# huttered40/capital

Hardware: AMD Instinct MI355X
Metric: TFLOP/s (whole node) Cholesky n=65536, algorithmic n^3/3, recursive cholinv factor(), inputs resident in HBM (higher is better)
Workload: dtype f64

## Files before the change

### capital_amd/capi.py

```python
import ctypes as C
import os

import numpy as np
import torch

_HERE = os.path.dirname(os.path.abspath(__file__))
LIB_PATH = os.environ.get("CAPITAL_HIP_LIB", os.path.join(_HERE, "libcapital_hip.so"))

NOTRANS, TRANS = 0, 1
LEFT, RIGHT = 0, 1
LOWER, UPPER = 0, 1
NONUNIT, UNIT = 0, 1
RECT, UPPERTRI, LOWERTRI = 0, 1, 2

_i64, _dbl, _int, _vp = C.c_int64, C.c_double, C.c_int, C.c_void_p

_SIGS = {
    "capi_dgemm": [_int, _int, _i64, _i64, _i64, _dbl, _vp, _i64, _vp, _i64, _dbl, _vp, _i64],
    "capi_dsyrk": [_int, _int, _i64, _i64, _dbl, _vp, _i64, _dbl, _vp, _i64],
    "capi_dgemmt": [_int, _int, _int, _i64, _i64, _dbl, _vp, _i64, _vp, _i64, _dbl, _vp, _i64],
    "capi_dsyrk_panel32": [_i64, _i64, _dbl, _vp, _dbl, _vp, _i64],
    "capi_dtrmm_right_panel32": [_i64, _i64, _dbl, _vp, _i64, _vp, _i64, _vp, _i64],
    "capi_dtrmm": [_int, _int, _int, _int, _i64, _i64, _dbl, _vp, _i64, _vp, _i64],
    "capi_dtrmm_oop": [_int, _int, _int, _int, _i64, _i64, _dbl, _vp, _i64, _vp, _i64, _vp, _i64],
    "capi_dtrmm_acc": [_int, _int, _int, _int, _i64, _i64, _dbl, _vp, _i64, _vp, _i64, _dbl, _vp, _i64],
    "capi_dtrsm": [_int, _int, _int, _int, _i64, _i64, _dbl, _vp, _i64, _vp, _i64],
    "capi_dpotrf": [_int, _i64, _vp, _i64],
    "capi_dtrtri": [_int, _int, _i64, _vp, _i64],
    "capi_dpotrf_trtri": [_i64, _vp, _i64, _vp, _i64],
    "capi_dgram_equilibrate_shift": [_i64, _vp, _i64, _i64, _dbl, _vp, _vp],
    "capi_dtri_rescale": [_i64, _vp, _i64, _vp, _i64, _vp, _vp],
    "capi_dgemtn_ts": [_i64, _i64, _i64, _dbl, _vp, _i64, _vp, _i64, _dbl, _vp, _i64],
    "capi_dresid_ts": [_i64, _i64, _i64, _vp, _i64, _vp, _i64, _vp, _i64, _vp, _i64, _vp],
    "capi_dtrmm_thin": [_int, _int, _i64, _i64, _i64, _dbl, _vp, _i64, _i64, _vp, _i64, _dbl, _vp, _i64],
    "capi_dresid_sym": [_i64, _i64, _vp, _i64, _vp, _i64, _vp, _i64, _vp, _i64, _vp],
    "capi_get_info": [C.POINTER(_int)],
    "capi_reset_info": [],
    "capi_serialize": [_int, _int, _vp, _i64, _i64, _vp, _i64, _i64] + [_i64] * 8,
    "capi_serialize_shape": [_int, _int, _int, _vp, _i64, _i64, _vp, _i64, _i64] + [_i64] * 8,
    "capi_dlacpy": [_int, _i64, _i64, _vp, _i64, _vp, _i64],
    "capi_dgeadd": [_int, _i64, _i64, _dbl, _vp, _i64, _dbl, _vp, _i64],
    "capi_dtrizero": [_int, _i64, _vp, _i64],
    "capi_daxpby": [_i64, _dbl, _vp, _vp],
    "capi_remove_triangle": [C.c_char, _vp, _i64, _i64, _i64, _i64, _i64],
    "capi_block_to_cyclic": [_vp, _vp, _i64, _i64, _i64],
    "capi_block_to_cyclic_full": [_vp, _vp, _i64, _i64, _i64],
    "capi_cyclic_to_block": [_vp, _vp, _i64, _i64, _i64],
# ... 162 lines not shown
```

### capital_amd/csrc/gemm_f64.hip

```cpp
#include "capi_internal.h"
#include "gemm_plan.h"
#include <type_traits>

extern "C" int capi_internal_copy2d(capi_handle_t h, int64_t m, int64_t n, const double* A, int64_t lda, double* B, int64_t ldb);

typedef double d4_t __attribute__((ext_vector_type(4)));
typedef double d2_t __attribute__((ext_vector_type(2)));

namespace {

constexpr int NTHREADS = 256;
using gemm_plan::BK, gemm_plan::SK;
template <int TS> struct tile_cfg {
  static constexpr int TILE_LDS = TS * SK;
  static constexpr int STAGE_LDS = 2 * TILE_LDS;
  static constexpr int NQ = TS / 32;
  static constexpr int SUB = TS / 32;
};
constexpr int GROUP_M = 8;
template <int TS> __device__ __forceinline__ int rc_r(int tid, int q) { return 16 * ((tid >> 6) * (TS / 64) + (q >> 1)) + 2 * (tid & 7); }
__device__ __forceinline__ int rc_k(int tid, int q) { return 8 * (q & 1) + ((tid >> 3) & 7); }

struct GemmArgs {
  const double* A;
// ... 457 lines not shown
}

template <bool AK, bool BKC>
__global__ __launch_bounds__(NTHREADS, 2) void dtrmm_pair_kernel(const GemmArgs p) {
  constexpr int TS = 128, BM = TS, BN = TS, SUB = tile_cfg<TS>::SUB, NQ = tile_cfg<TS>::NQ;
  constexpr int NW = NQ * ((AK ? 1 : 2) + (BKC ? 1 : 2));
  constexpr int TILE_LDS = tile_cfg<TS>::TILE_LDS, STAGE_LDS = tile_cfg<TS>::STAGE_LDS;
  constexpr int kstep = BK;
  extern __shared__ __attribute__((aligned(16))) double lds[];
  const int tid = threadIdx.x;
  const int lane = tid & 63, wave = tid >> 6;
  const int r16 = lane & 15, g = lane >> 4;
  const int wm = wave & 1, wn = wave >> 1;
  stamp_begin(p);

  const int nblk = gridDim.x, bid = blockIdx.x;
  const int xcd = bid & 7, qq = nblk >> 3, rr = nblk & 7;
  const int pid = p.pid_base + (xcd < rr ? xcd * (qq + 1) : rr * (qq + 1) + (xcd - rr) * qq) + (bid >> 3);
  const bool left = p.tri_side == CAPI_LEFT;
  const int ntri = left ? p.tiles_m : p.tiles_n, nfree = left ? p.tiles_n : p.tiles_m, npair = ntri >> 1;
  int pb, fr;
  if (left) tile_of_dims(-1, npair, nfree, pid, pb, fr); else tile_of_dims(-1, nfree, npair, pid, fr, pb);
  const bool anchor0 = left ? !p.tri_eff_upper : (p.tri_eff_upper != 0);
  const bool maskA = left, maskB = !left;
  const bool keep_ge = left == (p.tri_eff_upper != 0);
  const int64_t ksa = AK ? kstep : (int64_t)kstep * p.lda, ksb = BKC ? kstep : (int64_t)kstep * p.ldb;
  const int64_t qsa = AK ? 32 * p.lda : 8 * p.lda;
  const int64_t qsa2 = AK ? 64 * p.lda : 16;
  const int64_t qsb = BKC ? 32 * p.ldb : 8 * p.ldb;
  const int64_t qsb2 = BKC ? 64 * p.ldb : 16;

  for (int ph = 0; ph < 2; ++ph) {
    const bool asc = (ph == 0) == anchor0;
    const int bt = asc ? pb : ntri - 1 - pb;
    const int ti = left ? bt : fr, tj = left ? fr : bt;
    const int i0 = ti * BM, j0 = tj * BN, d0 = left ? i0 : j0;
    const int klo = anchor0 ? 0 : d0, khi = anchor0 ? d0 + TS : p.K;
    const int ntk = (khi - klo) / kstep;
    const int tb0 = (d0 - klo) / BK, tb1 = tb0 + TS / BK;

    d4_t acc[SUB][SUB];
#pragma unroll
    for (int a = 0; a < SUB; ++a)
#pragma unroll
      for (int c = 0; c < SUB; ++c) acc[a][c] = (d4_t){0.0, 0.0, 0.0, 0.0};

    const double* const fa0 = AK ? p.A + (int64_t)(i0 + (tid >> 3)) * p.lda + klo + 2 * (tid & 7)
                              : p.A + (int64_t)(klo + rc_k(tid, 0)) * p.lda + i0 + rc_r<TS>(tid, 0);
    const double* const fb0 = BKC ? p.B + (int64_t)(j0 + (tid >> 3)) * p.ldb + klo + 2 * (tid & 7)
                              : p.B + (int64_t)(klo + rc_k(tid, 0)) * p.ldb + j0 + rc_r<TS>(tid, 0);
    const double* fa = fa0;
    const double* fb = fb0;
    const int64_t sa = asc ? ksa : -ksa, sb = asc ? ksb : -ksb;
    const int dir = asc ? 1 : -1;
    int t = asc ? 0 : ntk - 1;

    d2_t ra[NQ], rb[NQ];
    {
      const int kf = klo + t * kstep;
      panel_load<TS, AK>(p.A, p.lda, i0, p.M, kf, khi, tid, 1, ra);
      panel_load<TS, BKC>(p.B, p.ldb, j0, p.N, kf, khi, tid, 1, rb);
      if (maskA && t >= tb0 && t < tb1) panel_mask<TS, AK>(i0, kf, tid, keep_ge, p.tri_unit, ra);
// ... 859 lines not shown
  CAPI_REQUIRE(h, n >= 0 && k >= 0 && n < (1LL << 31) && k < (1LL << 31), "dims");
  if (n == 0) return CAPI_OK;
  CAPI_REQUIRE(h, C && ldc >= n, "C/ldc");
  if (k > 0) {
    CAPI_REQUIRE(h, A && B, "null operand");
    CAPI_REQUIRE(h, lda >= (transA ? k : n) && ldb >= (transB ? n : k), "lda/ldb");
  }
  GemmArgs p{};
  p.A = A; p.B = B; p.C = C; p.lda = lda; p.ldb = ldb; p.ldc = ldc;
  p.M = (int)n; p.N = (int)n; p.K = (int)k; p.alpha = alpha; p.beta = beta;
  p.out_uplo = uplo; p.tri_side = -1;
  return launch_gemm(h, transA == CAPI_TRANS, transB == CAPI_NOTRANS, p, true);
}

int capi_dsyrk(capi_handle_t h, int uplo, int trans, int64_t n, int64_t k, double alpha,
               const double* A, int64_t lda, double beta, double* C, int64_t ldc) {
  CAPI_REQUIRE(h, h, "null handle");
  CAPI_REQUIRE(h, ok01(trans), "transpose code");
  return capi_dgemmt(h, uplo, trans, trans == CAPI_TRANS ? CAPI_NOTRANS : CAPI_TRANS, n, k, alpha, A, lda, A, lda, beta, C, ldc);
}

static int trmm_launch(capi_handle_t h, int side, int uplo, int trans, int diag, int64_t m, int64_t n, double alpha,
                       const double* T, int64_t ldt, const double* B, int64_t ldb, double beta, double* C, int64_t ldc,
                       size_t ws_held = 0) {
  CAPI_REQUIRE(h, h, "null handle");
  CAPI_REQUIRE(h, ok01(side) && ok01(uplo) && ok01(trans) && ok01(diag), "enum code");
  CAPI_REQUIRE(h, m >= 0 && n >= 0 && m < (1LL << 31) && n < (1LL << 31), "dims");
  if (m == 0 || n == 0) return CAPI_OK;
  const int64_t nt = side == CAPI_LEFT ? m : n;
  CAPI_REQUIRE(h, T && B && C && ldt >= nt && ldb >= m && ldc >= m, "operands");
  CAPI_REQUIRE(h, (const double*)C != B, "out-of-place trmm: C aliases B");
  GemmArgs p{};
  p.C = C; p.ldc = ldc; p.M = (int)m; p.N = (int)n; p.K = (int)nt; p.alpha = alpha; p.beta = beta;
  p.out_uplo = -1;
  p.tri_side = side;
  p.tri_eff_upper = ((uplo == CAPI_UPPER) != (trans == CAPI_TRANS));
  p.tri_unit = diag == CAPI_UNIT;
  if (side == CAPI_RIGHT && diag == CAPI_NONUNIT && n >= 512 && n <= 4096 && m >= 64 * n) {
    void* w;
    int rc = capi_ws3_get(h, sizeof(double) * (size_t)n * (size_t)n, &w);
    if (rc != CAPI_OK) return rc;
    CAPI_HIP_CHECK(h, hipMemsetAsync(w, 0, sizeof(double) * (size_t)n * (size_t)n, h->stream));
    rc = capi_dlacpy(h, uplo == CAPI_UPPER ? 1 : 2, n, n, T, ldt, (double*)w, n);
    if (rc != CAPI_OK) return rc;
    T = (const double*)w;
    ldt = n;
    p.tri_dense = 1;
    const bool eff_upper = (uplo == CAPI_UPPER) != (trans == CAPI_TRANS);
    if (eff_upper && n % 256 == 0) {
      for (int64_t J = 0; J < n / 256; ++J) {
        GemmArgs q = p;
        q.N = 256;
        q.K = (int)(256 * (J + 1));
        q.tri_koff = (int)(256 * J);
        q.tri_block = 1;
        q.C = C + 256 * J * ldc;
        q.A = B; q.lda = ldb;
        q.B = trans == CAPI_NOTRANS ? T + 256 * J * ldt : T + 256 * J;
        q.ldb = ldt;
        int rc2 = launch_gemm(h, false, trans == CAPI_NOTRANS, q, ws_held == 0);
        if (rc2 != CAPI_OK) return rc2;
      }
      return CAPI_OK;
    }
  }
  if (side == CAPI_LEFT) {
    p.A = T; p.lda = ldt; p.B = B; p.ldb = ldb;
    return launch_gemm(h, trans == CAPI_TRANS, true, p, true, ws_held);
  } else {
    p.A = B; p.lda = ldb; p.B = T; p.ldb = ldt;
// ... 10 lines not shown
  const bool aligned = ((st | sb_ | sc_) & 1) == 0;
  if (batch > 1 && small_ok && aligned) {
    const int64_t nt = side == CAPI_LEFT ? m : n;
    GemmArgs p{};
    p.C = C; p.ldc = ldc; p.M = (int)m; p.N = (int)n; p.K = (int)nt; p.alpha = alpha; p.beta = 0.0;
    p.out_uplo = -1; p.tri_side = side;
    p.tri_eff_upper = ((uplo == CAPI_UPPER) != (trans == CAPI_TRANS));
    p.tri_unit = diag == CAPI_UNIT;
    p.batch = batch;
    if (side == CAPI_LEFT) { p.A = T; p.lda = ldt; p.sa = st; p.B = B; p.ldb = ldb; p.sb = sb_; p.sc = sc_; return launch_gemm(h, trans == CAPI_TRANS, true, p, true); }
    p.A = B; p.lda = ldb; p.sa = sb_; p.B = T; p.ldb = ldt; p.sb = st; p.sc = sc_;
    return launch_gemm(h, false, trans == CAPI_NOTRANS, p, true);
  }
  for (int b = 0; b < batch; ++b) {
    int rc = capi_dtrmm_oop(h, side, uplo, trans, diag, m, n, alpha, T + b * st, ldt, B + b * sb_, ldb, C + b * sc_, ldc);
    if (rc != CAPI_OK) return rc;
  }
  return CAPI_OK;
}

int capi_dtrmm_oop(capi_handle_t h, int side, int uplo, int trans, int diag, int64_t m, int64_t n, double alpha,
                   const double* T, int64_t ldt, const double* B, int64_t ldb, double* C, int64_t ldc) {
  return trmm_launch(h, side, uplo, trans, diag, m, n, alpha, T, ldt, B, ldb, 0.0, C, ldc);
}

int capi_dtrmm_acc(capi_handle_t h, int side, int uplo, int trans, int diag, int64_t m, int64_t n, double alpha,
                   const double* T, int64_t ldt, const double* B, int64_t ldb, double beta, double* C, int64_t ldc) {
  return trmm_launch(h, side, uplo, trans, diag, m, n, alpha, T, ldt, B, ldb, beta, C, ldc);
}

int capi_dtrmm(capi_handle_t h, int side, int uplo, int trans, int diag, int64_t m, int64_t n, double alpha,
               const double* T, int64_t ldt, double* B, int64_t ldb) {
  CAPI_REQUIRE(h, h, "null handle");
  if (m <= 0 || n <= 0) return m < 0 || n < 0 ? CAPI_EINVAL : CAPI_OK;
  void* ws;
  int rc = capi_ws_get(h, sizeof(double) * (size_t)m * (size_t)n, &ws);
  if (rc != CAPI_OK) return rc;
  rc = trmm_launch(h, side, uplo, trans, diag, m, n, alpha, T, ldt, B, ldb, 0.0, (double*)ws, m, (size_t)m * (size_t)n);
  if (rc != CAPI_OK) return rc;
  rc = capi_ws_get(h, sizeof(double) * (size_t)m * (size_t)n, &ws);
  if (rc != CAPI_OK) return rc;
  return capi_internal_copy2d(h, m, n, (const double*)ws, m, B, ldb);
}

int capi_dsyrk_panel32(capi_handle_t h, int64_t n, int64_t k, double alpha, const double* A32, double beta, double* C, int64_t ldc) {
  CAPI_REQUIRE(h, h, "null handle");
// ... 131 lines not shown
```

### capital_amd/csrc/gemm_plan.h

```cpp
#ifndef CAPITAL_GEMM_PLAN_H_
#define CAPITAL_GEMM_PLAN_H_

#include <cstddef>
#include <cstdint>
#include <cstdio>

#include "capital_hip.h"

namespace gemm_plan {

constexpr int BK = 16;
constexpr int SK = BK + 2;
constexpr int ST = 32, SKC = 256, SQK = 64, SLD = ST + 2;
constexpr int TSK_W = 256;

inline int64_t cdiv(int64_t a, int64_t b) { return (a + b - 1) / b; }

struct Product {
  int M = 0, N = 0, K = 0;
  int out_uplo = -1;
  int tri_side = -1;
  int tri_eff_upper = 0, tri_dense = 0, tri_block = 0, tri_koff = 0;
  bool alpha_zero = false;
  double beta = 0.0;
  int batch = 0;
  bool ak = false, bkc = false;
  bool a_is_b = false;
  bool same_ld = false;
  bool a_vec = false, b_vec = false;
  bool a_tiled = false, c_tiled = false;
  bool ws_for_slab = true;
};
struct Device { int num_cu = 256; int stream_cu = 0; };
struct Modes { int rounds_mode = 0, pair_mode = 1, pair_rounds = 0, pair_rounds_min = 0; };
struct Overrides { int force_ts = 0; int force_small = -1; };

enum class Path { none, scale, trmm_ts32, gram_blocks, gram_ts, small, tile, pair, refused };
enum class Reduce { none, narrow, wide };
inline const char* path_name(Path p) {
// ... 143 lines not shown
      r.k_per_split = (int)kps;
      r.k_rotate = !tri;
      r.slab_ld = p.M;
      r.slab_stride = (int64_t)p.M * p.N;
      r.reduce = Reduce::narrow;
    }
  }
  const int per_round = 2 * ncu;
  const bool use_rounds = r.ts == 128 && r.splitk == 1 && !tri && per_round % 16 == 0 && p.batch <= 1 && r.ntiles >= 2 * per_round &&
                          (p.out_uplo < 0 ? (mode.rounds_mode & 1) != 0 : ((mode.rounds_mode & 2) != 0 && r.order));
  if (r.ts == 128 && r.splitk == 1 && !tri) {
    const int rem = r.ntiles % per_round;
    if (r.ntiles >= 2 * per_round && rem > 0 && rem <= (3 * per_round) / 4) r.tail128 = rem;
  }
  const int ntiles_all = r.ntiles;
  r.ntiles -= r.tail128;
  r.blocks = (int64_t)r.ntiles * r.splitk;
  r.per_launch = use_rounds ? per_round : r.blocks;
  r.lds_bytes = sizeof(double) * 2 * 2 * (size_t)r.ts * SK;
  r.variant = vi + (r.ts == 128 ? 0 : 4);
  r.share_den = (double)ntiles_all * r.splitk;
  const int ntri = p.tri_side == CAPI_LEFT ? r.tiles_m : r.tiles_n, nfree = p.tri_side == CAPI_LEFT ? r.tiles_n : r.tiles_m;
  const int64_t wgs = (int64_t)(ntri / 2) * nfree;
  if (mode.pair_mode && tri && !p.tri_dense && !p.tri_block && p.tri_koff == 0 && r.ts == 128 && r.splitk == 1 && p.beta == 0.0 &&
      p.batch <= 1 && p.M % 128 == 0 && p.N % 128 == 0 && p.K % 128 == 0 && p.a_vec && p.b_vec && (ntri & 1) == 0 && wgs % per_round == 0 &&
      (mode.pair_mode > 1 || wgs <= 4 * per_round || (mode.pair_rounds && p.K >= mode.pair_rounds_min))) {
    r.path = Path::pair;
    r.blocks = wgs;
    r.per_launch = mode.pair_rounds && wgs > per_round && p.K >= mode.pair_rounds_min ? per_round : wgs;
    r.variant = vi + 16;
    r.share_den = (double)wgs;
  }
  return r;
}

inline int format(char* buf, size_t n, const Product& p, const Device& d, const Modes& m, const Overrides& o, const Plan& r) {
  static const char* const reduce_names[] = {"none", "narrow", "wide"};
  return snprintf(buf, n,
                  "M=%d N=%d K=%d out_uplo=%d tri_side=%d tri_eff_upper=%d tri_dense=%d tri_block=%d tri_koff=%d alpha_zero=%d beta=%.17g "
                  "batch=%d ak=%d bkc=%d a_is_b=%d same_ld=%d a_vec=%d b_vec=%d a_tiled=%d c_tiled=%d ws_for_slab=%d num_cu=%d stream_cu=%d "
                  "rounds_mode=%d pair_mode=%d pair_rounds=%d pair_rounds_min=%d force_ts=%d force_small=%d -> path=%s ts=%d splitk=%d "
                  "k_per_split=%d k_rotate=%d order=%d share_ab=%d slab_stride=%lld tiles_m=%d tiles_n=%d ntiles=%d blocks=%lld "
                  "per_launch=%lld launches=%lld grid_y=%d tail128=%d reduce=%s lds=%zu variant=%d share_den=%.17g est_us=%.1f small_est_us=%.1f",
                  p.M, p.N, p.K, p.out_uplo, p.tri_side, p.tri_eff_upper, p.tri_dense, p.tri_block, p.tri_koff, (int)p.alpha_zero, p.beta,
                  p.batch, (int)p.ak, (int)p.bkc, (int)p.a_is_b, (int)p.same_ld, (int)p.a_vec, (int)p.b_vec, (int)p.a_tiled, (int)p.c_tiled,
                  (int)p.ws_for_slab, d.num_cu, d.stream_cu, m.rounds_mode, m.pair_mode, m.pair_rounds, m.pair_rounds_min, o.force_ts,
                  o.force_small, path_name(r.path), r.ts, r.splitk, r.k_per_split, r.k_rotate, r.order, r.share_ab, (long long)r.slab_stride,
// ... 8 lines not shown
```

### capital_amd/csrc/movement.hip

```cpp
#include "capi_internal.h"

namespace {

__device__ __host__ inline int64_t st_offset(int st, int64_t x, int64_t y, int64_t dimY) {
  if (st == CAPI_RECT) return x * dimY + y;
  if (st == CAPI_UPPERTRI) return ((x * (x + 1)) >> 1) + y;
  return x * dimY + y - (x * (x + 1) / 2);
}

__global__ void serialize_kernel(int shape, int ss, int ds, const double* __restrict__ src, int64_t sdimY, double* __restrict__ dst,
                                 int64_t ddimY, int64_t ssx, int64_t ssy, int64_t dsx, int64_t dsy, int64_t rangeX,
                                 int64_t rangeY) {
  const int64_t y = (int64_t)blockIdx.x * 1024 + threadIdx.x;
  const bool lower = shape == CAPI_LOWERTRI, upper = shape == CAPI_UPPERTRI;
  for (int64_t i = blockIdx.y; i < rangeX; i += gridDim.y) {
    int64_t so, d_o, cnt;
    if (lower) {
      so = st_offset(ss, ssx + i, ssy + i, sdimY);
      d_o = st_offset(ds, dsx + i, dsy + i, ddimY);
      cnt = rangeY - i;
    } else {
      so = st_offset(ss, ssx + i, ssy, sdimY);
      d_o = st_offset(ds, dsx + i, dsy, ddimY);
      cnt = upper ? i + 1 : rangeY;
    }
    if (y >= cnt) continue;
    double v[4];
#pragma unroll
    for (int q = 0; q < 4; ++q) v[q] = src[so + (y + 256 * q < cnt ? y + 256 * q : y)];
#pragma unroll
    for (int q = 0; q < 4; ++q)
      if (y + 256 * q < cnt) dst[d_o + y + 256 * q] = v[q];
  }
}

__global__ void lacpy_kernel(int part, int64_t m, int64_t n, const double* __restrict__ A, int64_t lda, double* __restrict__ B,
                             int64_t ldb) {
  const int64_t i = (int64_t)blockIdx.x * blockDim.x + threadIdx.x;
  const int64_t j0 = (int64_t)blockIdx.y * 8;
  if (i >= m) return;
#pragma unroll
  for (int q = 0; q < 8; ++q) {
    const int64_t j = j0 + q;
    if (j >= n) break;
    if (part == 1 && i > j) continue;
    if (part == 2 && i < j) continue;
    B[i + j * ldb] = A[i + j * lda];
  }
}

typedef double d2m_t __attribute__((ext_vector_type(2)));
template <bool VEC>
__global__ __launch_bounds__(256) void copy2d_kernel(int64_t m, int64_t n, const double* __restrict__ A, int64_t lda, double* __restrict__ B, int64_t ldb) {
  const int64_t i = ((int64_t)blockIdx.x * 256 + threadIdx.x) * (VEC ? 2 : 1);
  if (i >= m) return;
  for (int64_t j0 = (int64_t)blockIdx.y * 8; j0 < n; j0 += (int64_t)gridDim.y * 8) {
    if (VEC) {
      d2m_t v[8];
#pragma unroll
      for (int q = 0; q < 8; ++q) v[q] = *(const d2m_t*)(A + i + (j0 + q < n ? j0 + q : j0) * lda);
#pragma unroll
      for (int q = 0; q < 8; ++q)
        if (j0 + q < n) *(d2m_t*)(B + i + (j0 + q) * ldb) = v[q];
    } else {
      double v[8];
#pragma unroll
      for (int q = 0; q < 8; ++q) v[q] = A[i + (j0 + q < n ? j0 + q : j0) * lda];
#pragma unroll
      for (int q = 0; q < 8; ++q)
        if (j0 + q < n) B[i + (j0 + q) * ldb] = v[q];
    }
  }
}

// ... 161 lines not shown

void pad_lens(int64_t dimX, int64_t dimY, int64_t gdimX, int64_t gdimY, int64_t px, int64_t py, int64_t PX, int64_t PY,
              int64_t* padX, int64_t* padY) {
  *padX = (((gdimX % PX != 0) && ((dimX - 1) * PX + px >= gdimX)) ? dimX - 1 : dimX);
  *padY = (((gdimY % PY != 0) && ((dimY - 1) * PY + py >= gdimY)) ? dimY - 1 : dimY);
}

inline dim3 grid2(int64_t rows, int64_t cols) { return dim3((unsigned)cdiv(rows, 256), (unsigned)(cols < 65535 ? cols : 65535)); }

}

extern "C" {

int capi_serialize_shape(capi_handle_t h, int shape, int ss, int ds, const double* src, int64_t sdimX, int64_t sdimY, double* dst,
                         int64_t ddimX, int64_t ddimY, int64_t ssx, int64_t sex, int64_t ssy, int64_t sey, int64_t dsx, int64_t dex,
                         int64_t dsy, int64_t dey) {
  CAPI_REQUIRE(h, h, "null handle");
  CAPI_REQUIRE(h, ss >= 0 && ss <= 2 && ds >= 0 && ds <= 2 && shape >= 0 && shape <= 2, "structure code");
  CAPI_REQUIRE(h, (sex - ssx) == (dex - dsx) && (sey - ssy) == (dey - dsy), "source and destination ranges differ");
  (void)sdimX; (void)ddimX;
  const int64_t rangeX = sex - ssx, rangeY = sey - ssy;
  if (rangeX <= 0 || rangeY <= 0) return CAPI_OK;
  CAPI_REQUIRE(h, src && dst, "null matrix");
  hipLaunchKernelGGL(serialize_kernel, dim3((unsigned)cdiv(rangeY, 1024), (unsigned)(rangeX < 65535 ? rangeX : 65535)), dim3(256), 0, h->stream, shape, ss, ds, src, sdimY, dst, ddimY, ssx, ssy,
                     dsx, dsy, rangeX, rangeY);
  CAPI_HIP_CHECK(h, hipGetLastError());
  return CAPI_OK;
}

int capi_serialize(capi_handle_t h, int ss, int ds, const double* src, int64_t sdimX, int64_t sdimY, double* dst, int64_t ddimX,
                   int64_t ddimY, int64_t ssx, int64_t sex, int64_t ssy, int64_t sey, int64_t dsx, int64_t dex, int64_t dsy,
                   int64_t dey) {
  const int shape = (ss == CAPI_LOWERTRI || ds == CAPI_LOWERTRI) ? CAPI_LOWERTRI : ((ss == CAPI_UPPERTRI || ds == CAPI_UPPERTRI) ? CAPI_UPPERTRI : CAPI_RECT);
  return capi_serialize_shape(h, shape, ss, ds, src, sdimX, sdimY, dst, ddimX, ddimY, ssx, sex, ssy, sey, dsx, dex, dsy, dey);
}

__attribute__((visibility("hidden"))) int capi_internal_copy2d(capi_handle_t h, int64_t m, int64_t n, const double* A, int64_t lda, double* B, int64_t ldb) {
  if (m <= 0 || n <= 0 || (A == B && lda == ldb)) return CAPI_OK;
  if (lda == m && ldb == m && m * n >= (1 << 16) && (m > 8192 || n == 1)) {
    const int64_t total = m * n, cols = total / 8192, rest = total - cols * 8192;
    int rc = capi_internal_copy2d(h, 8192, cols, A, 8192, B, 8192);
    if (rc != CAPI_OK || rest == 0) return rc;
    return capi_internal_copy2d(h, rest, 1, A + cols * 8192, rest, B + cols * 8192, rest);
  }
  const bool vec = (((uintptr_t)A | (uintptr_t)B) & 15) == 0 && ((lda | ldb | m) & 1) == 0;
  const int64_t gx = cdiv(vec ? m / 2 : m, 256), gy = cdiv(n, 8);
  CAPI_REQUIRE(h, gx < (1LL << 31), "copy too tall");
  const dim3 grid((unsigned)gx, (unsigned)(gy < 65535 ? gy : 65535));
  if (vec) hipLaunchKernelGGL(copy2d_kernel<true>, grid, dim3(256), 0, h->stream, m, n, A, lda, B, ldb);
  else hipLaunchKernelGGL(copy2d_kernel<false>, grid, dim3(256), 0, h->stream, m, n, A, lda, B, ldb);
  CAPI_HIP_CHECK(h, hipGetLastError());
  return CAPI_OK;
}

int capi_dlacpy(capi_handle_t h, int part, int64_t m, int64_t n, const double* A, int64_t lda, double* B, int64_t ldb) {
  CAPI_REQUIRE(h, h, "null handle");
  CAPI_REQUIRE(h, part >= 0 && part <= 2 && m >= 0 && n >= 0, "args");
  if (m == 0 || n == 0) return CAPI_OK;
  CAPI_REQUIRE(h, A && B && lda >= m && ldb >= m, "operands");
  if (part == 0) return capi_internal_copy2d(h, m, n, A, lda, B, ldb);
  const int64_t gy = cdiv(n, 8);
  CAPI_REQUIRE(h, gy <= 65535, "n too large");
  hipLaunchKernelGGL(lacpy_kernel, dim3((unsigned)cdiv(m, 256), (unsigned)gy), dim3(256), 0, h->stream, part, m, n, A, lda, B, ldb);
  CAPI_HIP_CHECK(h, hipGetLastError());
  return CAPI_OK;
}

int capi_dgeadd(capi_handle_t h, int part, int64_t m, int64_t n, double alpha, const double* X, int64_t ldx, double beta, double* Y,
                int64_t ldy) {
  CAPI_REQUIRE(h, h, "null handle");
  CAPI_REQUIRE(h, part >= 0 && part <= 2 && m >= 0 && n >= 0, "args");
  if (m == 0 || n == 0) return CAPI_OK;
  CAPI_REQUIRE(h, X && Y && ldx >= m && ldy >= m, "operands");
  hipLaunchKernelGGL(geadd_kernel, grid2(m, n), dim3(256), 0, h->stream, part, m, n, alpha, X, ldx, beta, Y, ldy);
  CAPI_HIP_CHECK(h, hipGetLastError());
  return CAPI_OK;
}

int capi_dtrizero(capi_handle_t h, int keep_uplo, int64_t n, double* A, int64_t lda) {
  CAPI_REQUIRE(h, h, "null handle");
  CAPI_REQUIRE(h, (keep_uplo == 0 || keep_uplo == 1) && n >= 0, "args");
  if (n == 0) return CAPI_OK;
  CAPI_REQUIRE(h, A && lda >= n, "A/lda");
  hipLaunchKernelGGL(trizero_kernel, grid2(n, n), dim3(256), 0, h->stream, keep_uplo, n, A, lda);
  CAPI_HIP_CHECK(h, hipGetLastError());
  return CAPI_OK;
// ... 128 lines not shown
```

### capital_amd/src/alg/cholesky/cholinv/cholinv.h

```cpp
#ifndef CAPITAL_CHOLESKY_CHOLINV_H_
#define CAPITAL_CHOLESKY_CHOLINV_H_

#include "./../../alg.h"
#include "./../../matmult/summa/summa.h"
#include "./policy.h"

#pragma weak capi_dtrmm_thin
#pragma weak capi_dresid_ts
#pragma weak capi_dresid_sym

namespace cholesky {

template <class SerializePolicy = policy::cholinv::Serialize, class IntermediatesPolicy = policy::cholinv::SaveIntermediates,
          class BaseCasePolicy = policy::cholinv::NoReplication>
class cholinv : public SerializePolicy, public IntermediatesPolicy, public BaseCasePolicy {
public:
  using SP = SerializePolicy;
  using IP = IntermediatesPolicy;
  using BP = BaseCasePolicy;

  template <typename ScalarT, typename DimensionT>
  class info {
  public:
    using ScalarType = ScalarT;
    using DimensionType = DimensionT;
    using alg_type = cholinv<SerializePolicy, IntermediatesPolicy, BaseCasePolicy>;
    using SP = SerializePolicy;
    using IP = IntermediatesPolicy;
    using BP = BaseCasePolicy;
    info(const info& p) : complete_inv(p.complete_inv), split(p.split), bc_mult_dim(p.bc_mult_dim), dir(p.dir) {}
// ... 406 lines not shown
    ++args.num_levels;
    const U split2 = localDim - split1;
    const bool single = (t.d == 1 && t.c == 1);
    matmult::arena& ws = args.work;
    view R11i{Ri + start + start * ld, ld, split1, split1};
    view A12{R + start + (start + split1) * ld, ld, split1, split2};
    view A22{R + (start + split1) + (start + split1) * ld, ld, split2, split2};
    view R22i{Ri + (start + split1) + (start + split1) * ld, ld, split2, split2};
    view I12{Ri + start + (start + split1) * ld, ld, split1, split2};

    invoke(args, t, R, Ri, ld, start, split1, globalDim >> 1);
    if (wait_ev >= 0) CAPITAL_CHECK(capi_event_wait(h, wait_ev));
    if (start == 0 && args.input_lead > 0 && split1 == args.input_lead) CAPITAL_CHECK(capi_event_wait(h, EV_INPUT_MID));

    const bool top = (localDim == args.localDimension) && args.early_split == split1;
    if (top) CAPITAL_CHECK(capi_event_wait(h, EV_INPUT_REST));
    CRITTER_START(CI::trsm);
    int child_wait = -1;
    bool copy_deferred = false;
    const int64_t mark = ws.top;
    {
      view W{ws.take((int64_t)split1 * split2), split1, split1, split2};
      if (single) {
        CAPITAL_CHECK(capi_dtrmm_oop(h, CAPI_LEFT, CAPI_UPPER, CAPI_TRANS, CAPI_NONUNIT, split1, split2, 1.0, R11i.p, ld, A12.p, ld, W.p, W.ld));
      } else {
        view Tx{ws.take((int64_t)split1 * split1), split1, split1, split1};
        const int64_t np = matmult::summa::tri_count(split1);
        if ((t.x == t.y && !t.multipath) || !matmult::summa::packed_comm()) {
          CAPITAL_CHECK(capi_dlacpy(h, 0, split1, split1, R11i.p, ld, Tx.p, Tx.ld));
          util::transpose_raw(Tx.p, Tx.count(), ws.take(Tx.count()), t, matmult::summa::relay_space(t, Tx.count(), ws));
        } else if (t.x == t.y) {
          CAPITAL_CHECK(capi_dlacpy(h, 0, split1, split1, R11i.p, ld, Tx.p, Tx.ld));
          util::transpose_raw(nullptr, np, nullptr, t, matmult::summa::relay_space(t, np, ws));
        } else {
          double* pk = ws.take(np);
          matmult::summa::pack_tri(R11i, CAPI_UPPER, pk);
          util::transpose_raw(pk, np, ws.take(np), t, matmult::summa::relay_space(t, np, ws));
          matmult::summa::unpack_tri(pk, CAPI_UPPER, Tx);
        }
        matmult::summa::trmm(t, CAPI_LEFT, CAPI_UPPER, CAPI_TRANS, CAPI_NONUNIT, 1.0, Tx, A12, W, ws);
      }
      const U lead = split2 >> args.split;
      const bool a22_splits = !(((split2 * (U)t.d) <= args.bcDimension) || (lead < args.split));
      const bool la = single && a22_splits && lead > 0 && lookahead_min() >= 0 && (int64_t)split2 >= lookahead_min() && args.la_depth < lookahead_depth();
      const bool pack_now = top && !std::is_same<typename SP::structure, rect>::value;
      const bool copy_later = la && pack_now && !getenv("CAPITAL_PACK_AT_ONCE");
      if (!copy_later) CAPITAL_CHECK(capi_dlacpy(h, 0, split1, split2, W.p, W.ld, A12.p, ld));
// ... 32 lines not shown
        CAPITAL_CHECK(capi_dgemmt(h, CAPI_UPPER, CAPI_TRANS, CAPI_NOTRANS, split2, split1, -1.0, W.p, W.ld, W.p, W.ld, 1.0, A22.p, ld));
      } else {
        view Wx{ws.take(W.count()), split1, split1, split2};
        capital::dev_copy(Wx.p, W.p, W.count());
        util::transpose_raw(Wx.p, Wx.count(), ws.take(Wx.count()), t, matmult::summa::relay_space(t, Wx.count(), ws));
        matmult::summa::syrk(t, CAPI_UPPER, CAPI_TRANS, -1.0, W, Wx, 1.0, A22, ws);
      }
      if (pack_now && !packed_early) {
        CAPITAL_CHECK(capi_event_record(h, EV_TOP_R12));
        early_pack(EV_TOP_R12);
      }
      if (child_wait < 0) ws.top = mark;
      CRITTER_STOP(CI::tmu);
    }

    invoke(args, t, R, Ri, ld, start + split1, split2, split2 * (U)t.d, child_wait);
    if (child_wait >= 0) { --args.la_depth; ws.top = mark; }

    CRITTER_START(CI::tmu);
    if (!(!args.complete_inv && (globalDim == args.trueGlobalDimension))) {
      if (copy_deferred) CAPITAL_CHECK(capi_event_wait(h, EV_EARLY_PACK));
      const int64_t mark = ws.top;
      view W2{ws.take((int64_t)split1 * split2), split1, split1, split2};
      matmult::summa::trmm(t, CAPI_LEFT, CAPI_UPPER, CAPI_NOTRANS, CAPI_NONUNIT, 1.0, R11i, A12, W2, ws);
      if (single) {
        matmult::summa::trmm(t, CAPI_RIGHT, CAPI_UPPER, CAPI_NOTRANS, CAPI_NONUNIT, -1.0, R22i, W2, I12, ws);
      } else {
        view W3{ws.take(W2.count()), split1, split1, split2};
        matmult::summa::trmm(t, CAPI_RIGHT, CAPI_UPPER, CAPI_NOTRANS, CAPI_NONUNIT, -1.0, R22i, W2, W3, ws);
        CAPITAL_CHECK(capi_dlacpy(h, 0, split1, split2, W3.p, W3.ld, I12.p, ld));
      }
      ws.top = mark;
    }
    CRITTER_STOP(CI::tmu);
  }

  template <typename ArgType, typename CommType, typename U>
  static void base_case(ArgType& args, CommType&& t, double* R, double* Ri, U ld, U start, U localDim) {
    capi_handle_t h = capital::handle();
    ++args.num_base_cases;
    double* Rb = R + start + start * ld;
    double* Ib = Ri + start + start * ld;
    if (t.d == 1) {
      CAPITAL_CHECK(capi_dpotrf_trtri(h, localDim, Rb, ld, Ib, ld));
      return;
    }
    const int64_t d = (int64_t)t.d, L = (int64_t)localDim, agg = L * d;
    const int64_t span = ((start + localDim) != args.trueLocalDimension) ? agg : agg - (args.trueLocalDimension * d - args.trueGlobalDimension);
    constexpr bool packed_msg = !std::is_same<typename SP::structure, rect>::value;
// ... 96 lines not shown
```

### capital_amd/src/alg/matmult/summa/summa.h

```cpp
#ifndef CAPITAL_MATMULT_SUMMA_H_
#define CAPITAL_MATMULT_SUMMA_H_

#include "./../../alg.h"

namespace matmult {

struct arena {
  double* base = nullptr;
  int64_t cap = 0, top = 0;
  arena() = default;
  arena(const arena&) = delete;
  arena& operator=(const arena&) = delete;
  arena(arena&& o) noexcept : base(o.base), cap(o.cap), top(o.top) { o.base = nullptr; o.cap = o.top = 0; }
  arena& operator=(arena&& o) noexcept {
    if (this != &o) { release(); base = o.base; cap = o.cap; top = o.top; o.base = nullptr; o.cap = o.top = 0; }
    return *this;
  }
  ~arena() { release(); }
  void release() { capital::dev_free(base); base = nullptr; cap = top = 0; }
  void reserve(int64_t count) {
    if (count > cap) {
      capital::sync();
      capital::dev_free(base);
      base = capital::dev_alloc(count);
      cap = count;
    }
// ... 185 lines not shown
      if (!r.empty())
        for (size_t s = 0; s < steps; ++s) {
          stage(is_root(t, axis, s), src, land[s], r.c0, r.c1);
          bcast_axis(t, axis, s, land[s].p + r.c0 * land[s].ld, land[s].rows * r.width(), relay);
        }
      P.rec(pipe::EB + j);
    }
    return land;
  }
  template <typename CommType, typename RowsOf>
  static void depth_sum(CommType&& t, pipe& P, const chunks& plan, const view& acc, RowsOf&& rows_of, double* relay, arena& ws) {
    if (t.c == 1) { P.main(); return; }
    P.comm();
    double* half = depth_space(t, acc.rows * plan.widest(), ws);
    for (int j = 0; j < plan.nch; ++j) {
      const chunks::span r = plan.range(j);
      P.wait(pipe::EC + j);
      if (!r.empty()) allreduce_view(t, view{acc.p + r.c0 * acc.ld, acc.ld, rows_of(r.c1), r.width()}, half, relay, ws);
    }
    P.rec(pipe::ER);
    P.main(); P.wait(pipe::ER);
  }

  template <typename CommType>
  static void trmm(CommType&& t, int side, int uplo, int trans, int diag, double alpha, view T, view B, view Cout, arena& ws) {
    capi_handle_t h = capital::handle();
    const int64_t M = B.rows, N = B.cols;
    if (t.d == 1 && t.c == 1) {
      CAPITAL_CHECK(capi_dtrmm_oop(h, side, uplo, trans, diag, M, N, alpha, T.p, T.ld, B.p, B.ld, Cout.p, Cout.ld));
      return;
    }
    const bool eff_upper = (uplo == CAPI_UPPER) != (trans == CAPI_TRANS);
    if (t.d == 1 && colsplit() && (side == CAPI_LEFT || (eff_upper && trans == CAPI_NOTRANS))) {
      colsplit_run(t, N, side == CAPI_RIGHT, Cout.p, Cout.ld,
                   [&](int64_t c0, int64_t c1) {
                     double* Cj = Cout.p + c0 * Cout.ld;
                     if (side == CAPI_LEFT) {
                       CAPITAL_CHECK(capi_dtrmm_oop(h, side, uplo, trans, diag, M, c1 - c0, alpha, T.p, T.ld, B.p + c0 * B.ld, B.ld, Cj, Cout.ld));
                     } else {
                       if (c0 > 0)
                         CAPITAL_CHECK(capi_dgemm(h, CAPI_NOTRANS, CAPI_NOTRANS, M, c1 - c0, c0, alpha, B.p, B.ld, T.p + c0 * T.ld, T.ld, 0.0, Cj, Cout.ld));
                       CAPITAL_CHECK(capi_dtrmm_acc(h, side, uplo, trans, diag, M, c1 - c0, alpha, T.p + c0 + c0 * T.ld, T.ld, B.p + c0 * B.ld, B.ld,
                                                    c0 > 0 ? 1.0 : 0.0, Cj, Cout.ld));
                     }
                   },
                   [&](int64_t) { return M; }, ws);
      return;
    }
    const int64_t mark = ws.top;
    const size_t steps = t.d > 1 ? t.d / t.c : 1;
    const bool piped_left = side == CAPI_LEFT;
    const bool piped_right = side == CAPI_RIGHT && eff_upper && trans == CAPI_NOTRANS && t.d > 1;
// ... 354 lines not shown
```

### include/capital_hip.h

```cpp
#ifndef CAPITAL_HIP_H_
#define CAPITAL_HIP_H_

#include <stddef.h>
#include <stdint.h>

#ifdef __cplusplus
extern "C" {
#endif

typedef struct capi_handle_s* capi_handle_t;
typedef struct capi_comm_s*   capi_comm_t;

enum capi_status {
  CAPI_OK = 0,
  CAPI_EINVAL = -1,
  CAPI_EHIP = -2,
  CAPI_ENOMEM = -3,
  CAPI_ECOMM = -4,
  CAPI_ENOTSPD = -5
};
enum { CAPI_NOTRANS = 0, CAPI_TRANS = 1 };
enum { CAPI_LEFT = 0, CAPI_RIGHT = 1 };
enum { CAPI_LOWER = 0, CAPI_UPPER = 1 };
enum { CAPI_NONUNIT = 0, CAPI_UNIT = 1 };
// ... 8 lines not shown
const char* capi_last_error(capi_handle_t h);
int  capi_malloc(capi_handle_t h, void** dptr, size_t bytes);
int  capi_free(capi_handle_t h, void* dptr);
int  capi_memset_async(capi_handle_t h, void* dptr, int value, size_t bytes);
int  capi_memcpy_h2d(capi_handle_t h, void* dst, const void* src, size_t bytes);
int  capi_memcpy_d2h(capi_handle_t h, void* dst, const void* src, size_t bytes);
int  capi_memcpy_d2d_async(capi_handle_t h, void* dst, const void* src, size_t bytes);
int  capi_sync(capi_handle_t h);
int  capi_reserve_workspace(capi_handle_t h, size_t bytes);
int  capi_trim_workspaces(capi_handle_t h);
int  capi_set_launch_rounds(capi_handle_t h, int on, int* was);
int  capi_reserve_cus(capi_handle_t h, int reserve);

int capi_dgemm(capi_handle_t h, int transA, int transB, int64_t m, int64_t n, int64_t k, double alpha,
               const double* A, int64_t lda, const double* B, int64_t ldb, double beta, double* C, int64_t ldc);
int capi_dsyrk(capi_handle_t h, int uplo, int trans, int64_t n, int64_t k, double alpha,
               const double* A, int64_t lda, double beta, double* C, int64_t ldc);
int capi_dgemmt(capi_handle_t h, int uplo, int transA, int transB, int64_t n, int64_t k, double alpha,
                const double* A, int64_t lda, const double* B, int64_t ldb, double beta, double* C, int64_t ldc);
int capi_dtrmm(capi_handle_t h, int side, int uplo, int trans, int diag, int64_t m, int64_t n, double alpha,
               const double* T, int64_t ldt, double* B, int64_t ldb);
int capi_dtrmm_oop(capi_handle_t h, int side, int uplo, int trans, int diag, int64_t m, int64_t n, double alpha,
                   const double* T, int64_t ldt, const double* B, int64_t ldb, double* C, int64_t ldc);
int capi_dtrmm_acc(capi_handle_t h, int side, int uplo, int trans, int diag, int64_t m, int64_t n, double alpha,
                   const double* T, int64_t ldt, const double* B, int64_t ldb, double beta, double* C, int64_t ldc);
int capi_dtrsm(capi_handle_t h, int side, int uplo, int trans, int diag, int64_t m, int64_t n, double alpha,
               const double* T, int64_t ldt, double* B, int64_t ldb);

int capi_dsyrk_panel32(capi_handle_t h, int64_t n, int64_t k, double alpha, const double* A32, double beta, double* C, int64_t ldc);
int capi_dtrmm_right_panel32(capi_handle_t h, int64_t m, int64_t n, double alpha, const double* T, int64_t ldt,
                             const double* B, int64_t ldb, double* C, int64_t ldc);
int capi_dpotrf(capi_handle_t h, int uplo, int64_t n, double* A, int64_t lda);
int capi_dtrtri(capi_handle_t h, int uplo, int diag, int64_t n, double* A, int64_t lda);
int capi_dpotrf_trtri(capi_handle_t h, int64_t n, double* A, int64_t lda, double* Rinv, int64_t ldi);
int capi_get_info(capi_handle_t h, int* info);
int capi_dgram_equilibrate_shift(capi_handle_t h, int64_t n, double* G, int64_t ldg, int64_t m_global, double shift_scale,
                                 double* dscale, double* rec);
int capi_dtri_rescale(capi_handle_t h, int64_t n, double* R, int64_t ldr, double* Rinv, int64_t ldi, const double* dscale, double* rec);
enum { CAPI_TS_MAX_RHS = 32 };
int capi_dgemtn_ts(capi_handle_t h, int64_t m, int64_t n, int64_t r, double alpha, const double* A, int64_t lda, const double* B, int64_t ldb,
                   double beta, double* C, int64_t ldc);
int capi_dresid_ts(capi_handle_t h, int64_t m, int64_t n, int64_t r, const double* A, int64_t lda, const double* X, int64_t ldx,
                   const double* B, int64_t ldb, double* Rout, int64_t ldr, double* colnorm2);
int capi_dtrmm_thin(capi_handle_t h, int shape, int trans, int64_t m, int64_t n, int64_t r, double alpha,
                    const double* T, int64_t ldt, int64_t col0, const double* B, int64_t ldb, double beta, double* C, int64_t ldc);
int capi_dresid_sym(capi_handle_t h, int64_t n, int64_t r, const double* A, int64_t lda, const double* X, int64_t ldx,
// ... 68 lines not shown
```

Measured before the change: 55.15.

## Add clean-triangle TRMM path and faster serialize/lacpy copy kernels

Adds a capi_dtrmm_oop_clean entry for callers whose triangle already holds explicit zeros. It skips the workspace memset+lacpy densification and disables band masking in the trmm kernel, and it lets the pair path accept such triangles. Cholinv's single-device trmm calls now use it. The serialize and lacpy kernels are rewritten to process several columns per block with wider per-thread work, plus vectorized 2-wide loads. The risk is wrong results if a caller passes a triangle whose other half is not actually zero.

```diff
diff --git a/capital_amd/capi.py b/capital_amd/capi.py
--- a/capital_amd/capi.py
+++ b/capital_amd/capi.py
@@ -23,6 +23,7 @@
     "capi_dtrmm_right_panel32": [_i64, _i64, _dbl, _vp, _i64, _vp, _i64, _vp, _i64],
     "capi_dtrmm": [_int, _int, _int, _int, _i64, _i64, _dbl, _vp, _i64, _vp, _i64],
     "capi_dtrmm_oop": [_int, _int, _int, _int, _i64, _i64, _dbl, _vp, _i64, _vp, _i64, _vp, _i64],
+    "capi_dtrmm_oop_clean": [_int, _int, _int, _int, _i64, _i64, _dbl, _vp, _i64, _vp, _i64, _vp, _i64],
     "capi_dtrmm_acc": [_int, _int, _int, _int, _i64, _i64, _dbl, _vp, _i64, _vp, _i64, _dbl, _vp, _i64],
     "capi_dtrsm": [_int, _int, _int, _int, _i64, _i64, _dbl, _vp, _i64, _vp, _i64],
     "capi_dpotrf": [_int, _i64, _vp, _i64],
diff --git a/capital_amd/csrc/gemm_f64.hip b/capital_amd/csrc/gemm_f64.hip
--- a/capital_amd/csrc/gemm_f64.hip
+++ b/capital_amd/csrc/gemm_f64.hip
@@ -503,7 +503,8 @@
   int pb, fr;
   if (left) tile_of_dims(-1, npair, nfree, pid, pb, fr); else tile_of_dims(-1, nfree, npair, pid, fr, pb);
   const bool anchor0 = left ? !p.tri_eff_upper : (p.tri_eff_upper != 0);
-  const bool maskA = left, maskB = !left;
+  const bool band = !p.tri_dense;
+  const bool maskA = left && band, maskB = !left && band;
   const bool keep_ge = left == (p.tri_eff_upper != 0);
   const int64_t ksa = AK ? kstep : (int64_t)kstep * p.lda, ksb = BKC ? kstep : (int64_t)kstep * p.ldb;
   const int64_t qsa = AK ? 32 * p.lda : 8 * p.lda;
@@ -518,7 +519,7 @@
     const int i0 = ti * BM, j0 = tj * BN, d0 = left ? i0 : j0;
     const int klo = anchor0 ? 0 : d0, khi = anchor0 ? d0 + TS : p.K;
     const int ntk = (khi - klo) / kstep;
-    const int tb0 = (d0 - klo) / BK, tb1 = tb0 + TS / BK;
+    const int tb0 = band ? (d0 - klo) / BK : 0, tb1 = band ? tb0 + TS / BK : 0;
 
     d4_t acc[SUB][SUB];
 #pragma unroll
@@ -1424,9 +1425,10 @@
 
 static int trmm_launch(capi_handle_t h, int side, int uplo, int trans, int diag, int64_t m, int64_t n, double alpha,
                        const double* T, int64_t ldt, const double* B, int64_t ldb, double beta, double* C, int64_t ldc,
-                       size_t ws_held = 0) {
+                       size_t ws_held = 0, bool clean = false) {
   CAPI_REQUIRE(h, h, "null handle");
   CAPI_REQUIRE(h, ok01(side) && ok01(uplo) && ok01(trans) && ok01(diag), "enum code");
+  CAPI_REQUIRE(h, !clean || diag == CAPI_NONUNIT, "a clean triangle carries its own diagonal");
   CAPI_REQUIRE(h, m >= 0 && n >= 0 && m < (1LL << 31) && n < (1LL << 31), "dims");
   if (m == 0 || n == 0) return CAPI_OK;
   const int64_t nt = side == CAPI_LEFT ? m : n;
@@ -1438,16 +1440,19 @@
   p.tri_side = side;
   p.tri_eff_upper = ((uplo == CAPI_UPPER) != (trans == CAPI_TRANS));
   p.tri_unit = diag == CAPI_UNIT;
+  if (clean) p.tri_dense = gemm_plan::TRI_DENSE_CALLER;
   if (side == CAPI_RIGHT && diag == CAPI_NONUNIT && n >= 512 && n <= 4096 && m >= 64 * n) {
-    void* w;
-    int rc = capi_ws3_get(h, sizeof(double) * (size_t)n * (size_t)n, &w);
-    if (rc != CAPI_OK) return rc;
-    CAPI_HIP_CHECK(h, hipMemsetAsync(w, 0, sizeof(double) * (size_t)n * (size_t)n, h->stream));
-    rc = capi_dlacpy(h, uplo == CAPI_UPPER ? 1 : 2, n, n, T, ldt, (double*)w, n);
-    if (rc != CAPI_OK) return rc;
-    T = (const double*)w;
-    ldt = n;
-    p.tri_dense = 1;
+    if (!clean) {
+      void* w;
+      int rc = capi_ws3_get(h, sizeof(double) * (size_t)n * (size_t)n, &w);
+      if (rc != CAPI_OK) return rc;
+      CAPI_HIP_CHECK(h, hipMemsetAsync(w, 0, sizeof(double) * (size_t)n * (size_t)n, h->stream));
+      rc = capi_dlacpy(h, uplo == CAPI_UPPER ? 1 : 2, n, n, T, ldt, (double*)w, n);
+      if (rc != CAPI_OK) return rc;
+      T = (const double*)w;
+      ldt = n;
+      p.tri_dense = gemm_plan::TRI_DENSE_COPY;
+    }
     const bool eff_upper = (uplo == CAPI_UPPER) != (trans == CAPI_TRANS);
     if (eff_upper && n % 256 == 0) {
       for (int64_t J = 0; J < n / 256; ++J) {
@@ -1504,6 +1509,11 @@
 int capi_dtrmm_oop(capi_handle_t h, int side, int uplo, int trans, int diag, int64_t m, int64_t n, double alpha,
                    const double* T, int64_t ldt, const double* B, int64_t ldb, double* C, int64_t ldc) {
   return trmm_launch(h, side, uplo, trans, diag, m, n, alpha, T, ldt, B, ldb, 0.0, C, ldc);
+}
+
+int capi_dtrmm_oop_clean(capi_handle_t h, int side, int uplo, int trans, int diag, int64_t m, int64_t n, double alpha,
+                         const double* T, int64_t ldt, const double* B, int64_t ldb, double* C, int64_t ldc) {
+  return trmm_launch(h, side, uplo, trans, diag, m, n, alpha, T, ldt, B, ldb, 0.0, C, ldc, 0, true);
 }
 
 int capi_dtrmm_acc(capi_handle_t h, int side, int uplo, int trans, int diag, int64_t m, int64_t n, double alpha,
diff --git a/capital_amd/csrc/gemm_plan.h b/capital_amd/csrc/gemm_plan.h
--- a/capital_amd/csrc/gemm_plan.h
+++ b/capital_amd/csrc/gemm_plan.h
@@ -4,6 +4,7 @@
 #include <cstddef>
 #include <cstdint>
 #include <cstdio>
+#include <initializer_list>
 
 #include "capital_hip.h"
 
@@ -15,6 +16,8 @@
 constexpr int TSK_W = 256;
 
 inline int64_t cdiv(int64_t a, int64_t b) { return (a + b - 1) / b; }
+
+constexpr int TRI_DENSE_COPY = 1, TRI_DENSE_CALLER = 2;
 
 struct Product {
   int M = 0, N = 0, K = 0;
@@ -204,7 +207,7 @@
   r.share_den = (double)ntiles_all * r.splitk;
   const int ntri = p.tri_side == CAPI_LEFT ? r.tiles_m : r.tiles_n, nfree = p.tri_side == CAPI_LEFT ? r.tiles_n : r.tiles_m;
   const int64_t wgs = (int64_t)(ntri / 2) * nfree;
-  if (mode.pair_mode && tri && !p.tri_dense && !p.tri_block && p.tri_koff == 0 && r.ts == 128 && r.splitk == 1 && p.beta == 0.0 &&
+  if (mode.pair_mode && tri && (!p.tri_dense || p.tri_dense == TRI_DENSE_CALLER) && !p.tri_block && p.tri_koff == 0 && r.ts == 128 && r.splitk == 1 && p.beta == 0.0 &&
       p.batch <= 1 && p.M % 128 == 0 && p.N % 128 == 0 && p.K % 128 == 0 && p.a_vec && p.b_vec && (ntri & 1) == 0 && wgs % per_round == 0 &&
       (mode.pair_mode > 1 || wgs <= 4 * per_round || (mode.pair_rounds && p.K >= mode.pair_rounds_min))) {
     r.path = Path::pair;
diff --git a/capital_amd/csrc/movement.hip b/capital_amd/csrc/movement.hip
--- a/capital_amd/csrc/movement.hip
+++ b/capital_amd/csrc/movement.hip
@@ -8,48 +8,81 @@
   return x * dimY + y - (x * (x + 1) / 2);
 }
 
-__global__ void serialize_kernel(int shape, int ss, int ds, const double* __restrict__ src, int64_t sdimY, double* __restrict__ dst,
-                                 int64_t ddimY, int64_t ssx, int64_t ssy, int64_t dsx, int64_t dsy, int64_t rangeX,
-                                 int64_t rangeY) {
-  const int64_t y = (int64_t)blockIdx.x * 1024 + threadIdx.x;
+constexpr int SER_COLS = 8, SER_ROWS = 512;
+__global__ __launch_bounds__(256) void serialize_kernel(int shape, int ss, int ds, const double* __restrict__ src, int64_t sdimY,
+                                                        double* __restrict__ dst, int64_t ddimY, int64_t ssx, int64_t ssy, int64_t dsx,
+                                                        int64_t dsy, int64_t rangeX, int64_t rangeY) {
+  const int64_t yb = (int64_t)blockIdx.x * SER_ROWS, y0 = yb + threadIdx.x;
   const bool lower = shape == CAPI_LOWERTRI, upper = shape == CAPI_UPPERTRI;
-  for (int64_t i = blockIdx.y; i < rangeX; i += gridDim.y) {
-    int64_t so, d_o, cnt;
-    if (lower) {
-      so = st_offset(ss, ssx + i, ssy + i, sdimY);
-      d_o = st_offset(ds, dsx + i, dsy + i, ddimY);
-      cnt = rangeY - i;
+  for (int64_t i0 = (int64_t)blockIdx.y * SER_COLS; i0 < rangeX; i0 += (int64_t)gridDim.y * SER_COLS) {
+    const int64_t ilast = (i0 + SER_COLS < rangeX ? i0 + SER_COLS : rangeX) - 1;
+    const int64_t iref = lower ? i0 : ilast;
+    if (yb >= (lower ? rangeY - iref : (upper ? iref + 1 : rangeY))) continue;
+    const int64_t so_ref = lower ? st_offset(ss, ssx + iref, ssy + iref, sdimY) : st_offset(ss, ssx + iref, ssy, sdimY);
+    int64_t so[SER_COLS], d_o[SER_COLS], cnt[SER_COLS];
+#pragma unroll
+    for (int q = 0; q < SER_COLS; ++q) {
+      const int64_t i = i0 + q <= ilast ? i0 + q : iref;
+      if (lower) {
+        so[q] = st_offset(ss, ssx + i, ssy + i, sdimY);
+        d_o[q] = st_offset(ds, dsx + i, dsy + i, ddimY);
+        cnt[q] = rangeY - i;
+      } else {
+        so[q] = st_offset(ss, ssx + i, ssy, sdimY);
+        d_o[q] = st_offset(ds, dsx + i, dsy, ddimY);
+        cnt[q] = upper ? i + 1 : rangeY;
+      }
+      if (i0 + q > ilast) cnt[q] = 0;
+    }
+    double v[SER_COLS][SER_ROWS / 256];
+#pragma unroll
+    for (int q = 0; q < SER_COLS; ++q)
+#pragma unroll
+      for (int r = 0; r < SER_ROWS / 256; ++r) v[q][r] = src[y0 + 256 * r < cnt[q] ? so[q] + y0 + 256 * r : so_ref];
+#pragma unroll
+    for (int q = 0; q < SER_COLS; ++q)
+#pragma unroll
+      for (int r = 0; r < SER_ROWS / 256; ++r)
+        if (y0 + 256 * r < cnt[q]) dst[d_o[q] + y0 + 256 * r] = v[q][r];
+  }
+}
+
+typedef double d2m_t __attribute__((ext_vector_type(2)));
+template <bool VEC>
+__global__ __launch_bounds__(256) void lacpy_kernel(int part, int64_t m, int64_t n, const double* __restrict__ A, int64_t lda,
+                                                    double* __restrict__ B, int64_t ldb) {
+  const int64_t rb = (int64_t)blockIdx.x * 512, j0 = (int64_t)blockIdx.y * 8;
+  if (part == 1 ? rb > j0 + 7 : rb + 511 < j0) return;
+  const int64_t i0 = rb + (VEC ? 2 * threadIdx.x : threadIdx.x), i1 = i0 + (VEC ? 1 : 256);
+  if (i0 >= m) return;
+  const bool in1 = i1 < m;
+  double v0[8], v1[8];
+#pragma unroll
+  for (int q = 0; q < 8; ++q) {
+    const double* a = A + (j0 + q < n ? j0 + q : j0) * lda;
+    if (VEC) {
+      const d2m_t v = *(const d2m_t*)(a + i0);
+      v0[q] = v.x;
+      v1[q] = v.y;
     } else {
-      so = st_offset(ss, ssx + i, ssy, sdimY);
-      d_o = st_offset(ds, dsx + i, dsy, ddimY);
-      cnt = upper ? i + 1 : rangeY;
-    }
-    if (y >= cnt) continue;
-    double v[4];
-#pragma unroll
-    for (int q = 0; q < 4; ++q) v[q] = src[so + (y + 256 * q < cnt ? y + 256 * q : y)];
-#pragma unroll
-    for (int q = 0; q < 4; ++q)
-      if (y + 256 * q < cnt) dst[d_o + y + 256 * q] = v[q];
-  }
-}
-
-__global__ void lacpy_kernel(int part, int64_t m, int64_t n, const double* __restrict__ A, int64_t lda, double* __restrict__ B,
-                             int64_t ldb) {
-  const int64_t i = (int64_t)blockIdx.x * blockDim.x + threadIdx.x;
-  const int64_t j0 = (int64_t)blockIdx.y * 8;
-  if (i >= m) return;
+      v0[q] = a[i0];
+      v1[q] = a[in1 ? i1 : i0];
+    }
+  }
 #pragma unroll
   for (int q = 0; q < 8; ++q) {
     const int64_t j = j0 + q;
-    if (j >= n) break;
-    if (part == 1 && i > j) continue;
-    if (part == 2 && i < j) continue;
-    B[i + j * ldb] = A[i + j * lda];
-  }
-}
-
-typedef double d2m_t __attribute__((ext_vector_type(2)));
+    const bool w0 = j < n && (part == 1 ? i0 <= j : i0 >= j), w1 = j < n && in1 && (part == 1 ? i1 <= j : i1 >= j);
+    double* b = B + j * ldb;
+    if (VEC && w0 && w1) {
+      *(d2m_t*)(b + i0) = (d2m_t){v0[q], v1[q]};
+    } else {
+      if (w0) b[i0] = v0[q];
+      if (w1) b[i1] = v1[q];
+    }
+  }
+}
+
 template <bool VEC>
 __global__ __launch_bounds__(256) void copy2d_kernel(int64_t m, int64_t n, const double* __restrict__ A, int64_t lda, double* __restrict__ B, int64_t ldb) {
   const int64_t i = ((int64_t)blockIdx.x * 256 + threadIdx.x) * (VEC ? 2 : 1);
@@ -257,8 +290,10 @@
   const int64_t rangeX = sex - ssx, rangeY = sey - ssy;
   if (rangeX <= 0 || rangeY <= 0) return CAPI_OK;
   CAPI_REQUIRE(h, src && dst, "null matrix");
-  hipLaunchKernelGGL(serialize_kernel, dim3((unsigned)cdiv(rangeY, 1024), (unsigned)(rangeX < 65535 ? rangeX : 65535)), dim3(256), 0, h->stream, shape, ss, ds, src, sdimY, dst, ddimY, ssx, ssy,
-                     dsx, dsy, rangeX, rangeY);
+  const int64_t gx = cdiv(rangeY, SER_ROWS), gy = cdiv(rangeX, SER_COLS);
+  CAPI_REQUIRE(h, gx < (1LL << 31), "range too tall");
+  hipLaunchKernelGGL(serialize_kernel, dim3((unsigned)gx, (unsigned)(gy < 65535 ? gy : 65535)), dim3(256), 0, h->stream, shape, ss, ds, src, sdimY,
+                     dst, ddimY, ssx, ssy, dsx, dsy, rangeX, rangeY);
   CAPI_HIP_CHECK(h, hipGetLastError());
   return CAPI_OK;
 }
@@ -296,7 +331,10 @@
   if (part == 0) return capi_internal_copy2d(h, m, n, A, lda, B, ldb);
   const int64_t gy = cdiv(n, 8);
   CAPI_REQUIRE(h, gy <= 65535, "n too large");
-  hipLaunchKernelGGL(lacpy_kernel, dim3((unsigned)cdiv(m, 256), (unsigned)gy), dim3(256), 0, h->stream, part, m, n, A, lda, B, ldb);
+  const bool vec = (((uintptr_t)A | (uintptr_t)B) & 15) == 0 && ((lda | ldb | m) & 1) == 0;
+  const dim3 grid((unsigned)cdiv(m, 512), (unsigned)gy);
+  if (vec) hipLaunchKernelGGL(lacpy_kernel<true>, grid, dim3(256), 0, h->stream, part, m, n, A, lda, B, ldb);
+  else hipLaunchKernelGGL(lacpy_kernel<false>, grid, dim3(256), 0, h->stream, part, m, n, A, lda, B, ldb);
   CAPI_HIP_CHECK(h, hipGetLastError());
   return CAPI_OK;
 }
diff --git a/capital_amd/src/alg/cholesky/cholinv/cholinv.h b/capital_amd/src/alg/cholesky/cholinv/cholinv.h
--- a/capital_amd/src/alg/cholesky/cholinv/cholinv.h
+++ b/capital_amd/src/alg/cholesky/cholinv/cholinv.h
@@ -6,6 +6,7 @@
 #include "./policy.h"
 
 #pragma weak capi_dtrmm_thin
+#pragma weak capi_dtrmm_oop_clean
 #pragma weak capi_dresid_ts
 #pragma weak capi_dresid_sym
 
@@ -458,7 +459,7 @@
     {
       view W{ws.take((int64_t)split1 * split2), split1, split1, split2};
       if (single) {
-        CAPITAL_CHECK(capi_dtrmm_oop(h, CAPI_LEFT, CAPI_UPPER, CAPI_TRANS, CAPI_NONUNIT, split1, split2, 1.0, R11i.p, ld, A12.p, ld, W.p, W.ld));
+        matmult::summa::trmm_local(CAPI_LEFT, CAPI_UPPER, CAPI_TRANS, CAPI_NONUNIT, 1.0, R11i, A12, W, true);
       } else {
         view Tx{ws.take((int64_t)split1 * split1), split1, split1, split1};
         const int64_t np = matmult::summa::tri_count(split1);
@@ -537,9 +538,9 @@
       if (copy_deferred) CAPITAL_CHECK(capi_event_wait(h, EV_EARLY_PACK));
       const int64_t mark = ws.top;
       view W2{ws.take((int64_t)split1 * split2), split1, split1, split2};
-      matmult::summa::trmm(t, CAPI_LEFT, CAPI_UPPER, CAPI_NOTRANS, CAPI_NONUNIT, 1.0, R11i, A12, W2, ws);
+      matmult::summa::trmm(t, CAPI_LEFT, CAPI_UPPER, CAPI_NOTRANS, CAPI_NONUNIT, 1.0, R11i, A12, W2, ws, single);
       if (single) {
-        matmult::summa::trmm(t, CAPI_RIGHT, CAPI_UPPER, CAPI_NOTRANS, CAPI_NONUNIT, -1.0, R22i, W2, I12, ws);
+        matmult::summa::trmm(t, CAPI_RIGHT, CAPI_UPPER, CAPI_NOTRANS, CAPI_NONUNIT, -1.0, R22i, W2, I12, ws, true);
       } else {
         view W3{ws.take(W2.count()), split1, split1, split2};
         matmult::summa::trmm(t, CAPI_RIGHT, CAPI_UPPER, CAPI_NOTRANS, CAPI_NONUNIT, -1.0, R22i, W2, W3, ws);
diff --git a/capital_amd/src/alg/matmult/summa/summa.h b/capital_amd/src/alg/matmult/summa/summa.h
--- a/capital_amd/src/alg/matmult/summa/summa.h
+++ b/capital_amd/src/alg/matmult/summa/summa.h
@@ -2,6 +2,8 @@
 #define CAPITAL_MATMULT_SUMMA_H_
 
 #include "./../../alg.h"
+
+#pragma weak capi_dtrmm_oop_clean
 
 namespace matmult {
 
@@ -233,12 +235,17 @@
     P.main(); P.wait(pipe::ER);
   }
 
-  template <typename CommType>
-  static void trmm(CommType&& t, int side, int uplo, int trans, int diag, double alpha, view T, view B, view Cout, arena& ws) {
+  static void trmm_local(int side, int uplo, int trans, int diag, double alpha, view T, view B, view Cout, bool clean) {
+    auto* f = clean && &capi_dtrmm_oop_clean ? capi_dtrmm_oop_clean : capi_dtrmm_oop;
+    CAPITAL_CHECK(f(capital::handle(), side, uplo, trans, diag, B.rows, B.cols, alpha, T.p, T.ld, B.p, B.ld, Cout.p, Cout.ld));
+  }
+
+  template <typename CommType>
+  static void trmm(CommType&& t, int side, int uplo, int trans, int diag, double alpha, view T, view B, view Cout, arena& ws, bool clean = false) {
     capi_handle_t h = capital::handle();
     const int64_t M = B.rows, N = B.cols;
     if (t.d == 1 && t.c == 1) {
-      CAPITAL_CHECK(capi_dtrmm_oop(h, side, uplo, trans, diag, M, N, alpha, T.p, T.ld, B.p, B.ld, Cout.p, Cout.ld));
+      trmm_local(side, uplo, trans, diag, alpha, T, B, Cout, clean);
       return;
     }
     const bool eff_upper = (uplo == CAPI_UPPER) != (trans == CAPI_TRANS);
diff --git a/include/capital_hip.h b/include/capital_hip.h
--- a/include/capital_hip.h
+++ b/include/capital_hip.h
@@ -54,6 +54,8 @@
                const double* T, int64_t ldt, double* B, int64_t ldb);
 int capi_dtrmm_oop(capi_handle_t h, int side, int uplo, int trans, int diag, int64_t m, int64_t n, double alpha,
                    const double* T, int64_t ldt, const double* B, int64_t ldb, double* C, int64_t ldc);
+int capi_dtrmm_oop_clean(capi_handle_t h, int side, int uplo, int trans, int diag, int64_t m, int64_t n, double alpha,
+                         const double* T, int64_t ldt, const double* B, int64_t ldb, double* C, int64_t ldc);
 int capi_dtrmm_acc(capi_handle_t h, int side, int uplo, int trans, int diag, int64_t m, int64_t n, double alpha,
                    const double* T, int64_t ldt, const double* B, int64_t ldb, double beta, double* C, int64_t ldc);
 int capi_dtrsm(capi_handle_t h, int side, int uplo, int trans, int diag, int64_t m, int64_t n, double alpha,
```

Result: no change. 55.34 (median of 6 runs) (+0.3%).
